# cosmir17/Scala-akka-tensorflow-sharetrade-helper

Hardware: AMD Instinct MI355X
Metric: env steps/sec (whole node) + episode return, 2x128 MLP Q-net at 1/2/4/8 MI355X (higher is better)
Workload: dtype bf16; 1 GPU; model=2x128 MLP Q-net (203->128->128->3), online DQN, Adam, global_batch=1835008, seq_len=201, parallelism=dp1, dp_gradient_sync=none, envs_per_gpu=1835008, hip_graph=True, graph_steps=16, kernel_chunk=64, step_kernel=ws, chunk_schedule=static

## Files before the change

### csrc/qstep_ws.hip

```cpp
#include "qstep.h"

#ifndef WS_STAMPS
#define WS_STAMPS 0
#endif
#ifndef WS_GSKIP
#define WS_GSKIP 0
#endif
#if WS_MARKS
#define WS_MARK(W, I) asm volatile(";@" #W " " #I);
#else
#define WS_MARK(W, I)
#endif
#ifndef WS_PD1
#define WS_PD1 8
#endif
#ifndef WS_NOPHIL
#define WS_NOPHIL 0
#endif
constexpr int WS_GXP = 2;
#ifndef WS_L2PRE
#define WS_L2PRE 4
#endif
#ifndef WS_WAIT_UNROLL
#define WS_WAIT_UNROLL -1
#endif
#ifndef WS_SLEEP
#define WS_SLEEP 1
#endif
#ifndef WS_ABORT_WORD
#define WS_ABORT_WORD 1
#endif
#ifndef WS_NOWB
#define WS_NOWB 0
#endif
#ifndef WS_NOPF
#define WS_NOPF 0
#endif
#ifndef WS_L1REP
#define WS_L1REP 1
#endif
#ifndef WS_L2REP
#define WS_L2REP 1
#endif
#ifndef WS_GST_MASK
#define WS_GST_MASK 0x7F
#endif
#ifndef WS_NS
#define WS_NS ws
#define WS_API(name) name
#endif

namespace st {
namespace WS_NS {

constexpr int NW = 8, NT = 64 * NW;
constexpr int ND = 4, NG = 4;
constexpr int C = 64;
constexpr int INP = 224, HP = 128;
constexpr int KX = 208;
constexpr int HWIN = 201;
constexpr int NSLOT = 4;
static_assert(NSLOT % ND == 0, "a data wave reuses its own slots (sequence q = ND k + d)");

constexpr int oW0 = 0;
constexpr int oW1 = oW0 + HP * KX * 2;
constexpr int oW2 = oW1 + HP * HP * 2;
constexpr int oB1 = oW2 + 5 * HP * 2;
constexpr int oB2 = oB1 + HP * 4;
constexpr int oSLOT = oB2 + 64;
constexpr int sX = 0, sH1 = sX + 16 * KX * 2, sH2 = sH1 + 16 * HP * 2, sDZ2 = sH2 + 16 * HP * 2,
              SLOT_BYTES = sDZ2 + 16 * HP * 2;
constexpr int oCTL = oSLOT + NSLOT * SLOT_BYTES;
constexpr int oST = oCTL + 64;
constexpr int LDS_BYTES = oST + ND * NSTAT * 4;
static_assert(LDS_BYTES <= 163840, "LDS budget");
static_assert(SLOT_BYTES % 16 == 0 && oSLOT % 16 == 0, "alignment");

ST_DEV int pi_pos4(int i, int q) { return 32 * (i >> 1) + 8 * q + 4 * (i & 1); }
ST_DEV int w1_off(int R, int s) { return R * HP + ((((s >> 3) ^ (2 * (R & 7)))) << 3) + (s & 7); }
ST_DEV int a_off(int r, int c) {
  return r * HP + ((((c >> 2) ^ ((4 * (r & 7)) | ((r >> 2) & 3)))) << 2) + (c & 3);
}

ST_DEV s8v zero_s8() { s8v z = {0, 0, 0, 0, 0, 0, 0, 0}; return z; }
ST_DEV s4v mask_bf(f4v v, s4v act) {
  return pk4(act[0] > 0 ? v[0] : 0.f, act[1] > 0 ? v[1] : 0.f, act[2] > 0 ? v[2] : 0.f, act[3] > 0 ? v[3] : 0.f);
}
ST_DEV s4v lo4(s8v v) { s4v r = {v[0], v[1], v[2], v[3]}; return r; }
ST_DEV s4v hi4(s8v v) { s4v r = {v[4], v[5], v[6], v[7]}; return r; }

#ifndef WS_PD2
#define WS_PD2 8
#endif
constexpr int PD2 = WS_PD2, NB2 = PD2 + 1;
template <int NPRE>
ST_DEV void layer2_pre(const bf16_t* W1p, int l16, int g4, s8v* A) {
#pragma unroll
  for (int j = 0; j < NPRE; ++j) A[j] = lds_ld8(W1p + w1_off(16 * (j & 7) + l16, 32 * (j >> 3) + 8 * g4));
}
template <int NPRE = 0>
ST_DEV void layer2(const bf16_t* W1p, int l16, int g4, const s8v* H, f4v* acc, const bf16_t* w2row, s8v* w2f,
                   const s8v* Apre = nullptr) {
  s8v A[NB2];
#pragma unroll
  for (int j = 0; j < NPRE; ++j) A[j] = Apre[j];
#pragma unroll
  for (int j = NPRE; j < PD2; ++j) A[j] = lds_ld8(W1p + w1_off(16 * (j & 7) + l16, 32 * (j >> 3) + 8 * g4));
  if (NPRE < PD2) __builtin_amdgcn_sched_group_barrier(0x100, PD2 - NPRE, 0);
#pragma unroll
  for (int j = 0; j < 32; ++j) {
    acc[j & 7] = mfma32(A[j % NB2], H[j >> 3], acc[j & 7]);
    __builtin_amdgcn_sched_group_barrier(0x008, 1, 0);
    if (j + PD2 < 32) {
      const int jn = j + PD2;
      A[jn % NB2] = lds_ld8(W1p + w1_off(16 * (jn & 7) + l16, 32 * (jn >> 3) + 8 * g4));
      __builtin_amdgcn_sched_group_barrier(0x100, 1, 0);
    } else if (j >= 32 - 4) {
      w2f[j - 28] = lds_ld8(w2row + 32 * (j - 28));
      __builtin_amdgcn_sched_group_barrier(0x100, 1, 0);
    }
  }
  __builtin_amdgcn_sched_barrier(0);
}

constexpr int SPIN_LIMIT = 1 << 24;
constexpr int CTL_ABORT = 12;
constexpr int CTL_NROUNDS = 13;
ST_DEV int cid_word(int r) { const int s = r & 3; return s == 0 ? 0 : (s == 1 ? 9 : (s == 2 ? 14 : 15)); }
constexpr int CID_SHIFT = 21, CID_MASK = (1 << CID_SHIFT) - 1;
ST_DEV void ws_fail(const QStepParams& p, int* ctl) {
  if ((threadIdx.x & 63) == 0) {
    __hip_atomic_store(ctl + CTL_ABORT, 1, __ATOMIC_RELAXED, __HIP_MEMORY_SCOPE_WORKGROUP);
    if (p.err != nullptr) atomicOr(p.err, 1u);
  }
}
template <typename Pred>
ST_DEV void ring_wait(const QStepParams& p, int* ctl, const int* w, Pred pred) {
#if WS_WAIT_UNROLL > 0
#pragma clang loop unroll_count(WS_WAIT_UNROLL)
#elif WS_WAIT_UNROLL == 0
#pragma clang loop unroll(disable)
#endif
  for (int spin = 0; !pred(lds_acq(w)); ++spin) {
    if (WS_ABORT_WORD && lds_acq(ctl + CTL_ABORT)) break;
    if (WS_SLEEP > 0) __builtin_amdgcn_s_sleep(WS_SLEEP);
    if (spin > SPIN_LIMIT) { ws_fail(p, ctl); break; }
  }
}

ST_DEV int* env_ptr(const QStepParams& p, int R, int e) {
  return reinterpret_cast<int*>(reinterpret_cast<char*>(p.env + (size_t)R * p.E) + (unsigned)e * 4u);
}
#undef ENV_I
#undef ENV_F
#define ENV_I(R, e) (*env_ptr(p, (R), (e)))
#define ENV_F(R, e) (*reinterpret_cast<float*>(env_ptr(p, (R), (e))))

ST_DEV bool wait_full_or_end(const QStepParams& p, int* ctl, int sa, int q) {
#pragma clang loop unroll(disable)
  for (int spin = 0;; ++spin) {
    if (lds_acq(ctl + 1 + sa) == q + 1) return false;
    const int n = lds_acq(ctl + CTL_NROUNDS);
    if (n != 0 && q / ND >= n - 1) return true;
    if (WS_ABORT_WORD && lds_acq(ctl + CTL_ABORT)) return true;
    __builtin_amdgcn_s_sleep(1);
    if (spin > SPIN_LIMIT) { ws_fail(p, ctl); return true; }
  }
}

template <int FEAT, bool DYN, bool KN, bool U16 = false>
__global__ void __launch_bounds__(NT, 1) qstep_ws_kernel(QStepParams p) {
  static_assert(!U16 || FEAT, "the tick bank serves the relative features (w / last - 1) only");
  extern __shared__ __attribute__((aligned(16))) char smem[];
  bf16_t* W0p = reinterpret_cast<bf16_t*>(smem + oW0);
  bf16_t* W1p = reinterpret_cast<bf16_t*>(smem + oW1);
  bf16_t* W2p = reinterpret_cast<bf16_t*>(smem + oW2);
  float* sB1 = reinterpret_cast<float*>(smem + oB1);
  float* sB2 = reinterpret_cast<float*>(smem + oB2);
  int* ctl = reinterpret_cast<int*>(smem + oCTL);
  float* sSt = reinterpret_cast<float*>(smem + oST);

  const int tid = threadIdx.x, lane = tid & 63, l16 = lane & 15, g4 = lane >> 4;
  const int wave = __builtin_amdgcn_readfirstlane(tid >> 6);
  const unsigned long long step = p.ctrl[0];
  const int nchunks = p.E / C;
  const int nmy = (nchunks - (int)blockIdx.x + (int)gridDim.x - 1) / (int)gridDim.x;
  const int xg = (int)blockIdx.x & 7, gx = (int)gridDim.x >> 3;
  auto static_chunk = [&](int k) {
    const int c = (int)blockIdx.x + k * (int)gridDim.x;
    return c < nchunks ? c : -1;
  };

#if defined(WS_PROLOGUE_REPS) && WS_PROLOGUE_REPS > 1
  for (int rep_ = 0; rep_ < WS_PROLOGUE_REPS; ++rep_) {
    __syncthreads();
#else
  {
#endif
   if (p.wimg != nullptr) {
    constexpr int NCH = (oSLOT - oW0) / 16;
    for (int j = wave; j * 64 < NCH; j += NT / 64) {
      const int c = j * 64 + lane;
      if (c < NCH)
        __builtin_amdgcn_global_load_lds((const __attribute__((address_space(1))) void*)(p.wimg + 16 * c),
                                         (__attribute__((address_space(3))) void*)(smem + oW0 + 1024 * j), 16, 0, 0);
    }
    __builtin_amdgcn_s_waitcnt(0xF70);
   } else {
    const bf16_t* w0 = p.wq + p.off_w0;
    for (int i = tid; i < HP * KX; i += NT) {
      const int r = i / KX, s = i % KX;
      W0p[i] = w0[r * INP + slot_col(s)];
    }
    const bf16_t* w1 = p.wq + p.off_w1;
    for (int i = tid; i < HP * HP; i += NT) {
      const int R = i >> 7, s = i & 127;
      W1p[w1_off(R, s)] = w1[R * HP + pi_unit(s)];
    }
    const bf16_t* w2 = p.wq + p.off_w2;
    for (int i = tid; i < 5 * HP; i += NT) {
      const int a = i >> 7, s = i & 127;
      W2p[i] = w2[a * HP + pi_unit(s)];
    }
    for (int i = tid; i < HP; i += NT) sB1[i] = p.wf[p.off_b1 + i];
    if (tid < 16) sB2[tid] = tid < 4 ? p.wf[p.off_b2 + tid] : 0.f;
   }
    if (tid < 16) ctl[tid] = 0;
    if (DYN && tid == 0) {
      int r = 0;
      while (r < 3 && static_chunk(r) >= 0) ++r;
      if (r < 3) ctl[CTL_NROUNDS] = r + 1;
    }
  }
  __syncthreads();

  if (wave < ND) {
    const int d = wave;
    float st_reward = 0.f, st_loss = 0.f, st_explore = 0.f, st_done = 0.f, st_fsum = 0.f, st_fsq = 0.f,
          st_qslot = 0.f;
    const float b2v[3] = {sB2[0], sB2[1], sB2[2]};

    int ck0 = DYN ? static_chunk(0) : (int)blockIdx.x, ck1 = DYN ? static_chunk(1) : 0, ck2 = DYN ? static_chunk(2) : 0;
    auto ring_chunk = [&](int r) {
      int v = 0;
      ring_wait(p, ctl, ctl + cid_word(r), [&](int w) { v = w; return (w >> CID_SHIFT) == (r & 0x3FF); });
      return (v & CID_MASK) - 1;
    };
    unsigned claim_v = 0u;
    bool claim_out = false, ended = DYN && ck2 < 0;
    unsigned* const head = DYN ? p.chunk_heads + 32 * xg : nullptr;
    auto env_of = [&](int k, int rel) {
      if (DYN) {
        const int c = rel == 0 ? ck0 : (rel == 1 ? ck1 : ck2);
        return max(c, 0) * C + 16 * d + l16;
      }
      return (min((int)blockIdx.x + k * (int)gridDim.x, nchunks - 1)) * C + 16 * d + l16;
    };
    int e_pos, e_sh, e_ep, n_pos, n_sh, n_ep;
    float e_b, e_val, e_rs, n_b, n_val, n_rs;
    float e_sc = 1.f, n_sc = 1.f;
#define WS_LOAD_ENV(K, REL, POS, B, SH, VAL, RS, EP, SC)                                          \
  {                                                                                              \
    const int e_ = env_of(K, REL);                                                               \
    POS = ENV_I(ER_POS, e_); B = ENV_F(ER_BUDGET, e_); SH = ENV_I(ER_SHARES, e_);                \
    VAL = ENV_F(ER_VALUE, e_); RS = ENV_F(ER_RET_SUM, e_); EP = ENV_I(ER_EPISODES, e_);          \
    if (U16) SC = p.tscale[e_];                                                                  \
  }
    float4 pa[6], pb[6];
    float pc[6];
    float4 pd = make_float4(0.f, 0.f, 0.f, 0.f);
    float pe = 0.f;
    float4 pl;
    uint4 ta[6];
    unsigned tb[6];
    uint2 td = make_uint2(0u, 0u);
    unsigned te = 0u;
    uint2 tl;
#define WS_LOAD_PRICES(K, REL, POS)                                                               \
  if (U16) {                                                                                     \
    const int e_ = env_of(K, REL);                                                               \
    const int pc_ = min(max((POS), 0), p.T - HWIN - 1);                                          \
    const unsigned* b_ = reinterpret_cast<const unsigned*>(p.ticks + (size_t)e_ * p.T16) + (pc_ >> 1); \
    __builtin_memcpy(&tl, b_ + 100, sizeof(tl));                                                 \
    _Pragma("unroll") for (int ks = 0; ks < 6; ++ks) {                                           \
      __builtin_memcpy(&ta[ks], b_ + 16 * ks + 4 * g4, sizeof(uint4));                           \
      tb[ks] = b_[16 * ks + 4 * g4 + 4];                                                         \
    }                                                                                            \
    if (g4 == 1 || g4 == 2) {                                                                    \
      __builtin_memcpy(&td, b_ + 94 + 2 * g4, sizeof(td));                                       \
      te = b_[96 + 2 * g4];                                                                      \
    }                                                                                            \
  } else {                                                                                       \
    const int e_ = env_of(K, REL);                                                               \
    const int pc_ = min(max((POS), 0), p.T - HWIN - 1);    \
    const float* b_ = p.prices4 + (size_t)e_ * p.T4 + (size_t)pc_;     \
    pl = ldu4(b_ + 200);                           \
    _Pragma("unroll") for (int ks = 0; ks < 6; ++ks) {                                           \
      const float* q_ = b_ + 32 * ks + 8 * g4;                                                   \
      pa[ks] = ldu4(q_);                                                                         \
      pb[ks] = ldu4(q_ + 4);                                                                     \
      pc[ks] = q_[8];                                                                            \
    }                                                                                            \
    if (g4 == 1 || g4 == 2) {                                                                    \
      const float* r_ = b_ + 188 + 4 * g4;                                                       \
      pd = ldu4(r_);                                                                             \
      pe = r_[4];                                                                                \
    }                                                                                            \
  }
    WS_LOAD_ENV(0, 0, e_pos, e_b, e_sh, e_val, e_rs, e_ep, e_sc)
    WS_LOAD_PRICES(0, 0, e_pos)
    WS_LOAD_ENV(1, 1, n_pos, n_b, n_sh, n_val, n_rs, n_ep, n_sc)

    unsigned long long* stamps = ((WS_STAMPS & 1) && p.stamps != nullptr && blockIdx.x == 0 && d == 0 && lane == 0)
                                     ? p.stamps : nullptr;
#define WS_STAMP(I) if ((WS_STAMPS & 1) && stamps) stamps[k * 16 + (I)] = __builtin_amdgcn_s_memtime(); WS_MARK(D, I)
#define WS_PIN(V) asm volatile("" ::"v"(V))
#define WS_SB() __builtin_amdgcn_sched_barrier(0)

    int w_e = -1, w_s = 0, w_pos = 0, w_ep = 0, w_act = 0;
    float w_b = 0.f, w_v = 0.f, w_rs = 0.f, w_fin = 0.f, w_rew = 0.f;
    bool w_done = false;
#define WS_WRITE_BACK()                                                                           \
  if (!WS_NOWB && g4 == 0 && w_e >= 0) {                                                         \
    ENV_F(ER_BUDGET, w_e) = w_b; ENV_I(ER_SHARES, w_e) = w_s; ENV_F(ER_VALUE, w_e) = w_v;        \
    ENV_I(ER_POS, w_e) = w_pos; ENV_F(ER_RET_SUM, w_e) = w_rs;                                   \
    ENV_I(ER_ACTION, w_e) = w_act; ENV_F(ER_REWARD, w_e) = w_rew;                                \
    if (w_done) { ENV_F(ER_LAST_FINAL, w_e) = w_fin; ENV_I(ER_EPISODES, w_e) = w_ep; }           \
  }
#define WS_WB_SET()                                                                               \
  {                                                                                              \
    const int np_ = pos + 1;                                                                     \
    w_e = e; w_act = act; w_rew = rew;                                                           \
    w_done = np_ >= p.T - HWIN;                                                                  \
    w_ep = w_done ? ep0 + 1 : ep0;                                                               \
    if (w_done) {                                                                                \
      w_fin = __fadd_rn(b2, __fmul_rn((float)s2, vnew));                                         \
      w_b = p.b0; w_s = p.s0; w_v = 0.f; w_pos = 0; w_rs = 0.f;                                  \
    } else {                                                                                     \
      w_b = b2; w_s = s2; w_v = vnew; w_pos = np_; w_rs = rs0 + rew;                             \
    }                                                                                            \
    WS_WRITE_BACK() w_e = -1;                                                                    \
  }

    for (int k = 0; DYN ? ck0 >= 0 : k < nmy; ++k) {
      WS_STAMP(0);
      const int chunk = DYN ? ck0 : (int)blockIdx.x + k * (int)gridDim.x;
      if (DYN && k >= 1) ck2 = __builtin_amdgcn_readfirstlane(ring_chunk(k + 2));
      const int e = chunk * C + 16 * d + l16;
      float lastw, vnew_w, last, vnew;
      unsigned shb = 0u;
      if (U16) {
        shb = (unsigned)(min(max(e_pos, 0), p.T - HWIN - 1) & 1) * 2u;
        const unsigned t01 = __builtin_amdgcn_alignbyte(tl.y, tl.x, shb);
        lastw = (float)(t01 & 0xFFFFu);
        vnew_w = (float)(t01 >> 16);
        last = __fmul_rn(lastw, e_sc);
        vnew = __fmul_rn(vnew_w, e_sc);
      } else {
        lastw = last = pl.x;
        vnew_w = vnew = pl.y;
      }
      float inv = 0.f, invn = 0.f;
      if (FEAT) {
        inv = __fdiv_rn(1.0f, lastw);
        invn = __fdiv_rn(1.0f, vnew_w);
      }
      auto fx = [&](float w) {
        return FEAT ? __fmaf_rn(w, inv, -1.0f) : w;
      };
      auto fxn = [&](float w) {
        return FEAT ? __fmaf_rn(w, invn, -1.0f) : w;
      };
      auto lo16f = [](unsigned v) { return (float)(v & 0xFFFFu); };
      auto hi16f = [](unsigned v) { return (float)(v >> 16); };
      s8v X[6], Xn[6];
#pragma unroll
      for (int ks = 0; ks < 6; ++ks) {
        if (U16) {
          const unsigned w0 = __builtin_amdgcn_alignbyte(ta[ks].y, ta[ks].x, shb),
                         w1 = __builtin_amdgcn_alignbyte(ta[ks].z, ta[ks].y, shb),
                         w2 = __builtin_amdgcn_alignbyte(ta[ks].w, ta[ks].z, shb),
                         w3 = __builtin_amdgcn_alignbyte(tb[ks], ta[ks].w, shb),
                         w4 = __builtin_amdgcn_alignbyte(0u, tb[ks], shb);
          const float f0 = lo16f(w0), f1 = hi16f(w0), f2 = lo16f(w1), f3 = hi16f(w1), f4 = lo16f(w2),
                      f5 = hi16f(w2), f6 = lo16f(w3), f7 = hi16f(w3), f8 = lo16f(w4);
          X[ks] = cat8(pk4(fx(f0), fx(f1), fx(f2), fx(f3)), pk4(fx(f4), fx(f5), fx(f6), fx(f7)));
          Xn[ks] = cat8(pk4(fxn(f1), fxn(f2), fxn(f3), fxn(f4)), pk4(fxn(f5), fxn(f6), fxn(f7), fxn(f8)));
        } else {
          X[ks] = cat8(pk4(fx(pa[ks].x), fx(pa[ks].y), fx(pa[ks].z), fx(pa[ks].w)),
                       pk4(fx(pb[ks].x), fx(pb[ks].y), fx(pb[ks].z), fx(pb[ks].w)));
          Xn[ks] = cat8(pk4(fxn(pa[ks].y), fxn(pa[ks].z), fxn(pa[ks].w), fxn(pb[ks].x)),
                        pk4(fxn(pb[ks].y), fxn(pb[ks].z), fxn(pb[ks].w), fxn(pc[ks])));
        }
      }
      s4v X6, Xn6;
      if (g4 == 0) {
        X6 = pk4(feat_budget(e_b, p.inv_b0, FEAT), feat_shares(e_sh, last, p.inv_b0, FEAT), 1.0f, fx(lastw));
        Xn6 = zero_s4();
      } else if (g4 < 3) {
        if (U16) {
          const unsigned v0 = __builtin_amdgcn_alignbyte(td.y, td.x, shb), v1 = __builtin_amdgcn_alignbyte(te, td.y, shb),
                         v2 = __builtin_amdgcn_alignbyte(0u, te, shb);
          const float f0 = lo16f(v0), f1 = hi16f(v0), f2 = lo16f(v1), f3 = hi16f(v1), f4 = lo16f(v2);
          X6 = pk4(fx(f0), fx(f1), fx(f2), fx(f3));
          Xn6 = pk4(fxn(f1), fxn(f2), fxn(f3), fxn(f4));
        } else {
          X6 = pk4(fx(pd.x), fx(pd.y), fx(pd.z), fx(pd.w));
          Xn6 = pk4(fxn(pd.y), fxn(pd.z), fxn(pd.w), fxn(pe));
        }
      } else {
        X6 = zero_s4();
        Xn6 = zero_s4();
      }
      const int pos = e_pos, sh0 = e_sh, ep0 = e_ep;
      const float bud0 = e_b, vprev = e_val, rs0 = e_rs;
      e_pos = n_pos; e_b = n_b; e_sh = n_sh; e_val = n_val; e_rs = n_rs; e_ep = n_ep; e_sc = n_sc;
      WS_PIN(X[5]); WS_PIN(Xn[5]); WS_PIN(X6);
      WS_SB();
      WS_STAMP(1);
      WS_WRITE_BACK()
      WS_LOAD_ENV(k + 2, 2, n_pos, n_b, n_sh, n_val, n_rs, n_ep, n_sc)
      if (DYN && d == 0 && !ended) {
        if (lane == 0) claim_v = atomicAdd(head, 1u);
        claim_out = true;
      }
      float u1 = u24((uint32_t)(p.env_offset + e)), u2 = u24((uint32_t)step);
      if (!WS_NOPHIL) policy_draw((uint32_t)(p.env_offset + e), step, p.key0, p.key1, u1, u2);
      f4v a1[8], a1n[8];
#pragma unroll
      for (int i = 0; i < 8; ++i) { a1[i] = zero4(); a1n[i] = zero4(); }
      {
        constexpr int PD1 = WS_PD1, NB1 = PD1 + 1;
        const bf16_t* w0b = W0p + l16 * KX + 8 * g4;
        for (int rep = 0; rep < WS_L1REP; ++rep) {
        s8v A[NB1];
#pragma unroll
        for (int j = 0; j < PD1; ++j) A[j] = lds_ld8(w0b + (j & 7) * 16 * KX + 32 * (j >> 3));
        __builtin_amdgcn_sched_group_barrier(0x100, PD1, 0);
#pragma unroll
        for (int j = 0; j < 48; ++j) {
          const int ks = j >> 3, i = j & 7;
          a1[i] = mfma32(A[j % NB1], X[ks], a1[i]);
          a1n[i] = mfma32(A[j % NB1], Xn[ks], a1n[i]);
          __builtin_amdgcn_sched_group_barrier(0x008, 2, 0);
          if (j + PD1 < 48) {
            const int jn = j + PD1;
            A[jn % NB1] = lds_ld8(w0b + (jn & 7) * 16 * KX + 32 * (jn >> 3));
            __builtin_amdgcn_sched_group_barrier(0x100, 1, 0);
          }
          __builtin_amdgcn_sched_group_barrier(0x002, 2, 0);
        }
        }
        WS_PIN(u1); WS_PIN(u2);
        WS_SB();
      }
      WS_STAMP(12);
      s4v w06[8];
#pragma unroll
      for (int i = 0; i < 8; ++i) {
        w06[i] = lds_ld4(W0p + (16 * i + l16) * KX + 192 + 4 * g4);
        a1[i] = mfma16(w06[i], X6, a1[i]);
      }
      s8v H1[4];
#pragma unroll
      for (int ks = 0; ks < 4; ++ks) H1[ks] = cat8(relu_bf(a1[2 * ks]), relu_bf(a1[2 * ks + 1]));
      f4v a2[8];
#pragma unroll
      for (int i = 0; i < 8; ++i) a2[i] = *reinterpret_cast<const f4v*>(sB1 + 16 * i + 4 * g4);
      WS_PIN(H1[3]); WS_PIN(a1n[7]);
      WS_SB();
      WS_STAMP(2);
      s8v A2pre[WS_L2PRE];
      layer2_pre<WS_L2PRE>(W1p, l16, g4, A2pre);
      const int q = ND * k + d;
      const int sl = q % NSLOT, round = q / NSLOT;
      ring_wait(p, ctl, ctl + 5 + sl, [&](int v) { return v >= NG * round; });
      WS_STAMP(3);
      char* sb = smem + oSLOT + sl * SLOT_BYTES;
      bf16_t* sx = reinterpret_cast<bf16_t*>(sb + sX);
      bf16_t* sh1 = reinterpret_cast<bf16_t*>(sb + sH1);
      bf16_t* sh2 = reinterpret_cast<bf16_t*>(sb + sH2);
      bf16_t* sz2 = reinterpret_cast<bf16_t*>(sb + sDZ2);
#pragma unroll
      for (int ks = 0; ks < 6; ++ks) *reinterpret_cast<s8v*>(sx + l16 * KX + 32 * ks + 8 * g4) = X[ks];
      if (g4 < 3) *reinterpret_cast<s4v*>(sx + l16 * KX + 192 + 4 * g4) = X6;
#pragma unroll
      for (int i = 0; i < 8; ++i)
        *reinterpret_cast<s4v*>(sh1 + a_off(l16, 16 * i + 4 * g4)) = (i & 1) ? hi4(H1[i >> 1]) : lo4(H1[i >> 1]);
      WS_SB();
      WS_STAMP(4);
      const bf16_t* w2row = W2p + min(l16, 4) * HP + 8 * g4;
      s8v w2f[4];
      layer2<WS_L2PRE>(W1p, l16, g4, H1, a2, w2row, w2f, A2pre);
      s8v H2[4];
#pragma unroll
      for (int ks = 0; ks < 4; ++ks) H2[ks] = cat8(relu_bf(a2[2 * ks]), relu_bf(a2[2 * ks + 1]));
#pragma unroll
      for (int i = 0; i < 8; ++i)
        *reinterpret_cast<s4v*>(sh2 + a_off(l16, 16 * i + 4 * g4)) = (i & 1) ? hi4(H2[i >> 1]) : lo4(H2[i >> 1]);
      WS_PIN(H2[3]);
      WS_SB();
      WS_STAMP(5);
      f4v qa = zero4();
#pragma unroll
      for (int ks = 0; ks < 4; ++ks) {
        const s8v a = w2f[ks];
        qa = mfma32(a, H2[ks], qa);
      }
      WS_PIN(qa);
      WS_SB();
      WS_STAMP(6);
      float b2 = 0.f, rew = 0.f, q0 = 0.f, q1 = 0.f, q2 = 0.f;
      int s2 = 0, act = 0;
      if (g4 == 0) {
        q0 = qa[0] + b2v[0];
        q1 = qa[1] + b2v[1];
        q2 = qa[2] + b2v[2];
        if (p.output_relu) { q0 = fmaxf(q0, 0.f); q1 = fmaxf(q1, 0.f); q2 = fmaxf(q2, 0.f); }
        const int greedy = argmax3(q0, q1, q2);
        const bool exploit = exploits(u1, p.eps, (KN && p.ramp_global) ? (float)step : (float)pos, p.inv_ramp);
        const int rnd = random_action(u2);
        act = exploit ? greedy : rnd;
        const Holding h2 = trade(act, trade_base(bud0, sh0, p.compat_env, p.b0, p.s0), vnew);
        b2 = h2.budget;
        s2 = h2.shares;
        rew = reward(bud0, sh0, vprev, b2, s2, vnew, p.reward_mode);
        Xn6 = pk4(feat_budget(b2, p.inv_b0, FEAT), feat_shares(s2, vnew, p.inv_b0, FEAT), 1.0f, fxn(vnew_w));
        st_explore += exploit ? 0.f : 1.f;
      }
      WS_WB_SET()
      WS_PIN(Xn6);
      WS_SB();
      WS_STAMP(7);
#pragma unroll
      for (int i = 0; i < 8; ++i) a1n[i] = mfma16(w06[i], Xn6, a1n[i]);
      s8v H1n[4];
#pragma unroll
      for (int ks = 0; ks < 4; ++ks) H1n[ks] = cat8(relu_bf(a1n[2 * ks]), relu_bf(a1n[2 * ks + 1]));
      WS_LOAD_PRICES(k + 1, 1, e_pos)
#pragma unroll
      for (int i = 0; i < 8; ++i) a2[i] = *reinterpret_cast<const f4v*>(sB1 + 16 * i + 4 * g4);
      WS_SB();
      for (int rep = 0; rep < WS_L2REP; ++rep) layer2(W1p, l16, g4, H1n, a2, w2row, w2f);
      s8v H2n[4];
#pragma unroll
      for (int ks = 0; ks < 4; ++ks) H2n[ks] = cat8(relu_bf(a2[2 * ks]), relu_bf(a2[2 * ks + 1]));
      f4v qn = zero4();
#pragma unroll
      for (int ks = 0; ks < 4; ++ks) {
        const s8v a = w2f[ks];
        qn = mfma32(a, H2n[ks], qn);
      }
      WS_PIN(qn);
      WS_SB();
      WS_STAMP(8);
      const bf16_t* zchunk = reinterpret_cast<const bf16_t*>(ctl + 10);
      s4v aw[8], h2m[8];
      auto dz_reads = [&]() {
// ... 7 lines not shown
      float dq = 0.f;
      int slot = 0;
      if (g4 == 0) {
        float4 tq = make_float4(0.f, 0.f, 0.f, 0.f);
        if (KN && p.qt != nullptr) tq = *reinterpret_cast<const float4*>(p.qt + ((size_t)e * 3 + act) * 4);
        float n0 = qn[0] + b2v[0], n1 = qn[1] + b2v[1], n2 = qn[2] + b2v[2];
        if (p.output_relu) { n0 = fmaxf(n0, 0.f); n1 = fmaxf(n1, 0.f); n2 = fmaxf(n2, 0.f); }
        float vnext;
        const int am = argmax3(n0, n1, n2, vnext);
        slot = p.target_compat ? am : act;
        if (KN && p.qt != nullptr) vnext = target_value(tq.x, tq.y, tq.z, am, p.target_compat || p.double_dqn);
        const float y = td_target(rew, KN ? p.reward_scale : 1.0f, p.gamma, vnext);
        const float qs = slot == 0 ? q0 : (slot == 1 ? q1 : q2);
        float diff;
        dq = td_dq(qs, y, p.loss_coef, p.td_clip, p.output_relu, diff);
        float fdone = 0.f, ndone = 0.f;
        if (pos + 1 >= p.T - HWIN) {
          fdone = __fadd_rn(b2, __fmul_rn((float)s2, vnew));
          ndone = 1.f;
        }
        st_reward += rew;
        st_loss += diff * diff;
        st_qslot += qs;
        st_done += ndone;
        st_fsum += fdone;
        st_fsq += fdone * fdone;
      }
      WS_SB();
      WS_STAMP(9);
      const s4v bq = g4 == 0 ? pk4(slot == 0 ? dq : 0.f, slot == 1 ? dq : 0.f, slot == 2 ? dq : 0.f, 0.f)
                             : zero_s4();
      s4v dz[8];
      f4v zt[8];
#pragma unroll
      for (int i = 0; i < 8; ++i) zt[i] = mfma16(aw[i], bq, zero4());
#pragma unroll
      for (int i = 0; i < 8; ++i) dz[i] = mask_pk(zt[i], h2m[i]);
      WS_PIN(dz[7]);
      WS_SB();
      WS_STAMP(10);
#pragma unroll
      for (int ks = 0; ks < 4; ++ks)
        *reinterpret_cast<s8v*>(sz2 + w1_off(l16, 32 * ks + 8 * g4)) = cat8(dz[2 * ks], dz[2 * ks + 1]);
      if (g4 == 0) *reinterpret_cast<s4v*>(sx + l16 * KX + 204) = bq;
      if (lane == 0) __hip_atomic_store(ctl + 1 + sl, q + 1, __ATOMIC_RELEASE, __HIP_MEMORY_SCOPE_WORKGROUP);
      if (DYN) {
        if (d == 0) {
          int c = -1;
          if (claim_out) {
            const unsigned cv = (unsigned)__builtin_amdgcn_readfirstlane((int)claim_v);
            const long long cc = 8ll * (3ll * gx + (long long)cv) + xg;
            c = cc < nchunks ? (int)cc : -1;
            claim_out = false;
          }
          const bool first_end = c < 0 && !ended;
          if (c < 0) ended = true;
          if (lane == 0) {
            if (first_end && ck2 >= 0)
              __hip_atomic_store(ctl + CTL_NROUNDS, k + 3 + 1, __ATOMIC_RELAXED, __HIP_MEMORY_SCOPE_WORKGROUP);
            __hip_atomic_store(ctl + cid_word(k + 3), (((k + 3) & 0x3FF) << CID_SHIFT) | (c + 1), __ATOMIC_RELEASE,
                               __HIP_MEMORY_SCOPE_WORKGROUP);
          }
        }
        ck0 = ck1;
        ck1 = ck2;
      }
      WS_SB();
      WS_STAMP(11);
    }
    WS_WRITE_BACK()
#undef WS_WRITE_BACK
#undef WS_WB_SET
#undef WS_LOAD_ENV
#undef WS_LOAD_PRICES
#undef WS_STAMP
    const float v[NSTAT - 1] = {st_reward, st_loss, st_explore, st_done, st_fsum, st_fsq, st_qslot};
#pragma unroll
    for (int s = 0; s < NSTAT - 1; ++s) {
      const float t = wave_sum(v[s]);
      if (lane == 0) sSt[d * NSTAT + s] = t;
    }
    if (lane == 0) sSt[d * NSTAT + NSTAT - 1] = 0.f;
    __syncthreads();
  } else {
    const int gw = wave - ND;
    f4v gW0[2][13], gW1[2][8], gW2[2];
    float gB1s[2] = {0.f, 0.f}, gB2s = 0.f;
    auto sum8 = [](const s8v& v) {
      float acc = 0.f;
#pragma unroll
      for (int j = 0; j < 8; ++j) acc += bf2f((bf16_t)v[j]);
      return acc;
    };
#pragma unroll
    for (int m = 0; m < 2; ++m) {
#pragma unroll
      for (int n = 0; n < 13; ++n) gW0[m][n] = zero4();
#pragma unroll
      for (int n = 0; n < 8; ++n) gW1[m][n] = zero4();
      gW2[m] = zero4();
    }
    s4v ones;
#pragma unroll
    for (int j = 0; j < 4; ++j) ones[j] = (l16 == 0) ? (short)0x3F80 : (short)0;
    const int r4 = 4 * g4 + (l16 >> 2), qq = l16 & 3;
    const bf16_t* zchunk = reinterpret_cast<const bf16_t*>(ctl + 10);
    const int nseq = ND * nmy;
    unsigned long long* gst = ((WS_STAMPS & 2) && p.stamps != nullptr && blockIdx.x == 0 && gw == 0 && lane == 0)
                                  ? p.stamps + (size_t)(nmy + 1) * 16 : nullptr;
    unsigned long long gts[7] = {0, 0, 0, 0, 0, 0, 0};
#define WS_GST(I) if ((WS_STAMPS & 2) && ((WS_GST_MASK >> (I)) & 1)) gts[I] = __builtin_amdgcn_s_memtime(); WS_MARK(G, I)
    int nseqv = DYN ? 0x7FFFFFF0 : nseq;
    for (int q = 0; q < nseqv; q += 2) {
      const int sa = q % NSLOT, sb = (q + 1) % NSLOT;
      WS_GST(0);
      if (DYN) {
        if (wait_full_or_end(p, ctl, sa, q)) {
          nseqv = q;
          continue;
        }
      } else {
        ring_wait(p, ctl, ctl + 1 + sa, [&](int v) { return v == q + 1; });
      }
      ring_wait(p, ctl, ctl + 1 + sb, [&](int v) { return v == q + 2; });
      WS_GST(1);
#if WS_GSKIP
      if (lane == 0) {
        __hip_atomic_fetch_add(ctl + 5 + sa, 1, __ATOMIC_RELEASE, __HIP_MEMORY_SCOPE_WORKGROUP);
        __hip_atomic_fetch_add(ctl + 5 + sb, 1, __ATOMIC_RELEASE, __HIP_MEMORY_SCOPE_WORKGROUP);
      }
      continue;
#endif
      const char* pa_ = smem + oSLOT + sa * SLOT_BYTES;
      const char* pb_ = smem + oSLOT + sb * SLOT_BYTES;
      const bf16_t *xa = reinterpret_cast<const bf16_t*>(pa_ + sX), *xb = reinterpret_cast<const bf16_t*>(pb_ + sX);
      const bf16_t *h1a = reinterpret_cast<const bf16_t*>(pa_ + sH1), *h1b = reinterpret_cast<const bf16_t*>(pb_ + sH1);
      const bf16_t *h2a = reinterpret_cast<const bf16_t*>(pa_ + sH2), *h2b = reinterpret_cast<const bf16_t*>(pb_ + sH2);
      const bf16_t *z2a = reinterpret_cast<const bf16_t*>(pa_ + sDZ2), *z2b = reinterpret_cast<const bf16_t*>(pb_ + sDZ2);
      auto tr8 = [&](const bf16_t* a, const bf16_t* b, int off) { return cat8(lds_tr4(a + off), lds_tr4(b + off)); };
      f4v c1a[2] = {zero4(), zero4()}, c1b[2] = {zero4(), zero4()};
#pragma unroll
      for (int ks = 0; ks < 4; ++ks) {
        const s8v aza = lds_ld8(z2a + w1_off(l16, 32 * ks + 8 * g4));
        const s8v azb = lds_ld8(z2b + w1_off(l16, 32 * ks + 8 * g4));
        const int R = 32 * ks + 4 * g4 + (l16 >> 2);
#pragma unroll
        for (int t = 0; t < 2; ++t) {
          const int col = pi_pos4(2 * gw + t, qq);
          const s8v wt = cat8(lds_tr4(W1p + w1_off(R, col)), lds_tr4(W1p + w1_off(R + 16, col)));
          c1a[t] = mfma32(aza, wt, c1a[t]);
          c1b[t] = mfma32(azb, wt, c1b[t]);
        }
      }
      s4v bowna[2], bownb[2];
#pragma unroll
      for (int t = 0; t < 2; ++t) {
        bowna[t] = lds_tr4(h1a + a_off(r4, 16 * (2 * gw + t) + 4 * qq));
        bownb[t] = lds_tr4(h1b + a_off(r4, 16 * (2 * gw + t) + 4 * qq));
      }
      constexpr int XD = WS_GXP;
      s8v bx[13];
#pragma unroll
      for (int n = 0; n < XD; ++n) bx[n] = tr8(xa, xb, r4 * KX + 16 * n + 4 * qq);
      WS_PIN(c1a[1]); WS_PIN(c1b[1]);
      WS_SB();
      WS_GST(2);
      s8v a0[2];
#pragma unroll
      for (int t = 0; t < 2; ++t) a0[t] = cat8(mask_pk(c1a[t], bowna[t]), mask_pk(c1b[t], bownb[t]));
      WS_PIN(a0[1]);
      WS_SB();
      WS_GST(3);
#pragma unroll
      for (int n = 0; n < 13; ++n) {
#pragma unroll
        for (int m = 0; m < 2; ++m) gW0[m][n] = mfma32(a0[m], bx[n], gW0[m][n]);
        __builtin_amdgcn_sched_group_barrier(0x008, 2, 0);
        if (n + XD < 13) {
          bx[n + XD] = tr8(xa, xb, r4 * KX + 16 * (n + XD) + 4 * qq);
          __builtin_amdgcn_sched_group_barrier(0x100, 2, 0);
        }
      }
      WS_PIN(gW0[1][12]);
      WS_SB();
      WS_GST(4);
      s8v a1[2];
#pragma unroll
      for (int m = 0; m < 2; ++m) a1[m] = tr8(z2a, z2b, w1_off(r4, pi_pos4(2 * gw + m, qq)));
#pragma unroll
      for (int m = 0; m < 2; ++m) gB1s[m] += sum8(a1[m]);
#pragma unroll
      for (int half = 0; half < 2; ++half) {
        s8v bh[4];
#pragma unroll
        for (int k = 0; k < 4; ++k) bh[k] = tr8(h1a, h1b, a_off(r4, 16 * (4 * half + k) + 4 * qq));
#pragma unroll
        for (int m = 0; m < 2; ++m)
#pragma unroll
          for (int k = 0; k < 4; ++k) gW1[m][4 * half + k] = mfma32(a1[m], bh[k], gW1[m][4 * half + k]);
      }
      {
        const s8v aq = qq == 0 ? tr8(xa, xb, r4 * KX + 204) : cat8(lds_tr4(zchunk), lds_tr4(zchunk));
        s8v bh2[2];
#pragma unroll
        for (int k = 0; k < 2; ++k) bh2[k] = tr8(h2a, h2b, a_off(r4, 16 * (2 * gw + k) + 4 * qq));
        if (lane == 0) {
          __hip_atomic_fetch_add(ctl + 5 + sa, 1, __ATOMIC_RELEASE, __HIP_MEMORY_SCOPE_WORKGROUP);
          __hip_atomic_fetch_add(ctl + 5 + sb, 1, __ATOMIC_RELEASE, __HIP_MEMORY_SCOPE_WORKGROUP);
        }
        WS_GST(5);
#pragma unroll
        for (int n = 0; n < 2; ++n) gW2[n] = mfma32(aq, bh2[n], gW2[n]);
        gB2s += sum8(aq);
      }
      WS_PIN(gW1[1][7]); WS_PIN(gB2s);
      WS_SB();
      WS_GST(6);
      if ((WS_STAMPS & 2) && gst) {
#pragma unroll
        for (int i = 0; i < 7; ++i) gst[8 * q + i] = gts[i];
      }
    }
    __syncthreads();
    auto put = [&](int idx, float v) {
      if (p.slab_bf16) {
        bf16_t* sbf = reinterpret_cast<bf16_t*>(p.slab);
        sbf[((size_t)(idx >> 5) * p.slab_rows + blockIdx.x) * 32 + (idx & 31)] = f2bf(v);
      } else {
        p.slab[(size_t)blockIdx.x * p.P + idx] = v;
      }
    };
#pragma unroll
    for (int m = 0; m < 2; ++m)
#pragma unroll
      for (int j = 0; j < 4; ++j) {
        const int u = 32 * gw + 16 * m + 4 * g4 + j;
#pragma unroll
        for (int n = 0; n < 13; ++n) put(p.off_w0 + u * INP + slot_col(16 * n + l16), gW0[m][n][j]);
#pragma unroll
        for (int n = 0; n < 8; ++n) put(p.off_w1 + u * HP + 16 * n + l16, gW1[m][n][j]);
      }
#pragma unroll
    for (int m = 0; m < 2; ++m) {
      float v = gB1s[m];
      v += __shfl_xor(v, 16, 64);
      v += __shfl_xor(v, 32, 64);
      if (g4 == 0) put(p.off_b1 + 32 * gw + 16 * m + l16, v);
    }
    {
      float v = gB2s;
      v += __shfl_xor(v, 16, 64);
      v += __shfl_xor(v, 32, 64);
      if (gw == 0 && g4 == 0 && l16 < 4) put(p.off_b2 + l16, v);
    }
#pragma unroll
    for (int n = 0; n < 2; ++n)
#pragma unroll
      for (int j = 0; j < 4; ++j) put(p.off_w2 + (4 * g4 + j) * HP + 16 * (2 * gw + n) + l16, gW2[n][j]);
  }
#undef WS_SB
#undef WS_PIN
#undef WS_GST
  if (tid < NSTAT) {
    float t = 0.f;
#pragma unroll
    for (int w = 0; w < ND; ++w) t += sSt[w * NSTAT + tid];
    p.stats[(size_t)blockIdx.x * NSTAT + tid] = t;
  }
  if (blockIdx.x == 0 && tid == 0) p.ctrl[1] = step + 1;
}

template <int FEAT, bool DYN, bool KN, bool U16 = false>
static hipError_t launch_f(const QStepParams& p, int grid, hipStream_t stream) {
  static bool attr = false;
  if (!attr) {
    hipError_t e = hipFuncSetAttribute((const void*)qstep_ws_kernel<FEAT, DYN, KN, U16>,
                                       hipFuncAttributeMaxDynamicSharedMemorySize, LDS_BYTES);
    if (e != hipSuccess) return e;
    attr = true;
  }
  hipLaunchKernelGGL((qstep_ws_kernel<FEAT, DYN, KN, U16>), dim3(grid), dim3(NT), LDS_BYTES, stream, p);
  return hipGetLastError();
}

__global__ void __launch_bounds__(256) ws_img_map_kernel(int* map, int off_w0, int off_w1, int off_w2, int off_b1,
                                                         int off_b2) {
  const int i = blockIdx.x * blockDim.x + threadIdx.x;
  if (i < HP * KX) map[off_w0 + (i / KX) * INP + slot_col(i % KX)] = oW0 / 2 + i;
  if (i < HP * HP) map[off_w1 + (i >> 7) * HP + pi_unit(i & 127)] = oW1 / 2 + w1_off(i >> 7, i & 127);
  if (i < 5 * HP) map[off_w2 + (i >> 7) * HP + pi_unit(i & 127)] = oW2 / 2 + i;
  if (i < HP) map[off_b1 + i] = -(oB1 / 4 + i) - 2;
  if (i < 4) map[off_b2 + i] = -(oB2 / 4 + i) - 2;
}

}
}

extern "C" int WS_API(st_qstep_ws_img_bytes)() { return st::WS_NS::oSLOT - st::WS_NS::oW0; }

extern "C" hipError_t WS_API(st_qstep_ws_img_map)(int* map, int off_w0, int off_w1, int off_w2, int off_b1, int off_b2,
                                                  hipStream_t stream) {
  using namespace st::WS_NS;
  static_assert(oW0 == 0 && (oSLOT - oW0) % 16 == 0, "image run");
  hipLaunchKernelGGL(ws_img_map_kernel, dim3((HP * KX + 255) / 256), dim3(256), 0, stream, map, off_w0, off_w1, off_w2,
                     off_b1, off_b2);
  return hipGetLastError();
}

extern "C" int WS_API(st_qstep_ws_lds_bytes)(int inp, int h1p, int h2p) {
  if (inp == st::WS_NS::INP && h1p == st::WS_NS::HP && h2p == st::WS_NS::HP) return st::WS_NS::LDS_BYTES;
  return -1;
}

extern "C" hipError_t WS_API(st_qstep_ws_launch)(const st::QStepParams* p, int inp, int h1p, int h2p, int grid,
                                                 hipStream_t stream) {
  using namespace st::WS_NS;
  if (inp != INP || h1p != HP || h2p != HP || p->H != HWIN) return hipErrorInvalidValue;
  if (p->E % C != 0 || grid < 1 || grid > p->E / C) return hipErrorInvalidValue;
  if (p->chunk_heads != nullptr && (grid % 8 != 0 || p->E / C >= (1 << CID_SHIFT) - 1)) return hipErrorInvalidValue;
  if (p->T < HWIN + 2 || p->T4 < p->T + 4) return hipErrorInvalidValue;
  if ((p->off_w0 | p->off_w1 | p->off_w2) & 7) return hipErrorInvalidValue;
  if (p->slab_bf16 && (p->slab_rows != grid || p->P % 32 != 0)) return hipErrorInvalidValue;
  const bool kn = p->qt != nullptr || p->reward_scale != 1.0f || p->ramp_global || p->double_dqn;
  if (p->ticks != nullptr) {
    if (!p->feat_mode || p->tscale == nullptr || p->T16 < p->T + 8 || p->T16 % 8) return hipErrorInvalidValue;
    if (kn) {
      if (p->chunk_heads != nullptr || (p->double_dqn && p->qt == nullptr)) return hipErrorInvalidValue;
      return launch_f<1, false, true, true>(*p, grid, stream);
    }
    if (p->chunk_heads != nullptr) return launch_f<1, true, false, true>(*p, grid, stream);
    return launch_f<1, false, false, true>(*p, grid, stream);
  }
  if (kn) {
    if (p->chunk_heads != nullptr || (p->double_dqn && p->qt == nullptr)) return hipErrorInvalidValue;
    return p->feat_mode ? launch_f<1, false, true>(*p, grid, stream) : launch_f<0, false, true>(*p, grid, stream);
  }
  if (p->chunk_heads != nullptr)
    return p->feat_mode ? launch_f<1, true, false>(*p, grid, stream) : launch_f<0, true, false>(*p, grid, stream);
  return p->feat_mode ? launch_f<1, false, false>(*p, grid, stream) : launch_f<0, false, false>(*p, grid, stream);
}
```

### sharetrade/ops/native.py

```python
from __future__ import annotations

import ctypes as C
import os
from typing import Optional

import torch

_HERE = os.path.dirname(os.path.abspath(__file__))
LIB_DIR = os.path.join(os.path.dirname(_HERE), "_native")
HIP_LIB_PATH = os.path.join(LIB_DIR, "libsharetrade_hip.so")

_lib: Optional[C.CDLL] = None


class NativeUnavailable(RuntimeError):
    pass


class QStepParams(C.Structure):
    _fields_ = [
        ("prices", C.c_void_p), ("prices4", C.c_void_p), ("env", C.c_void_p),
        ("wq", C.c_void_p), ("wf", C.c_void_p), ("slab", C.c_void_p), ("stats", C.c_void_p), ("ctrl", C.c_void_p),
        ("T", C.c_int), ("E", C.c_int), ("H", C.c_int), ("P", C.c_int), ("T4", C.c_int),
        ("off_w0", C.c_int), ("off_w1", C.c_int), ("off_b1", C.c_int), ("off_w2", C.c_int), ("off_b2", C.c_int),
        ("eps", C.c_float), ("inv_ramp", C.c_float), ("gamma", C.c_float), ("loss_coef", C.c_float),
        ("b0", C.c_float), ("inv_b0", C.c_float),
        ("s0", C.c_int), ("compat_env", C.c_int), ("target_compat", C.c_int), ("output_relu", C.c_int),
        ("feat_mode", C.c_int),
        ("key0", C.c_uint32), ("key1", C.c_uint32),
        ("env_offset", C.c_int),
        ("stamps", C.c_void_p),
        ("slab_bf16", C.c_int), ("slab_rows", C.c_int),
        ("chunk_heads", C.c_void_p),
        ("reward_mode", C.c_int), ("td_clip", C.c_float),
        ("err", C.c_void_p),
        ("reward_scale", C.c_float), ("ramp_global", C.c_int), ("qt", C.c_void_p), ("double_dqn", C.c_int),
        ("wimg", C.c_void_p),
        ("ticks", C.c_void_p), ("tscale", C.c_void_p), ("T16", C.c_int),
    ]


QTARGET_VARIANTS = {0: (4, 4), 1: (2, 8), 2: (1, 8), 3: (1, 16)}


class QTargetParams(C.Structure):
    _fields_ = [
        ("prices4", C.c_void_p), ("env", C.c_void_p), ("wt", C.c_void_p), ("qt", C.c_void_p),
        ("T", C.c_int), ("E", C.c_int), ("T4", C.c_int),
        ("off_w0", C.c_int), ("off_w1", C.c_int), ("off_b1", C.c_int), ("off_w2", C.c_int), ("off_b2", C.c_int),
        ("b0", C.c_float), ("inv_b0", C.c_float),
        ("s0", C.c_int), ("compat_env", C.c_int), ("output_relu", C.c_int), ("feat_mode", C.c_int),
        ("wimg", C.c_void_p),
        ("ticks", C.c_void_p), ("tscale", C.c_void_p), ("T16", C.c_int),
    ]


class OptimParams(C.Structure):
    _fields_ = [
        ("params", C.c_void_p), ("params_bf", C.c_void_p), ("mask", C.c_void_p), ("s1", C.c_void_p),
        ("s2", C.c_void_p), ("slab", C.c_void_p), ("grad", C.c_void_p), ("ctrl", C.c_void_p),
        ("stats", C.c_void_p), ("stat_acc", C.c_void_p),
        ("G", C.c_int), ("P", C.c_int), ("kind", C.c_int), ("mode", C.c_int), ("nstat", C.c_int),
        ("lr", C.c_float), ("beta1", C.c_float), ("beta2", C.c_float), ("eps", C.c_float), ("scale", C.c_float),
        ("tdelay", C.c_int), ("slab_bf16", C.c_int),
        ("chunk_heads", C.c_void_p),
        ("ema", C.c_void_p), ("ema_decay", C.c_float),
        ("img_map", C.c_void_p), ("img", C.c_void_p),
    ]


REWARD_MODES = {"absolute": 0, "relative": 1, "growth": 2}

ENV_ROWS = ("pos", "budget", "shares", "value", "ret_sum", "episodes", "last_final", "actions_out", "rewards_out")


AB_LIB_PATH = os.path.join(LIB_DIR, "libsharetrade_ab.so")
WRONG_RESULT_VARIANTS = frozenset({"gskip", "gskipst", "l1x2", "l2x2", "nopf", "nowb", "nophil"})
_ab_lib: Optional[C.CDLL] = None


def ab_builds_enabled() -> bool:
    return os.environ.get("SHARETRADE_AB_BUILDS", "") not in ("", "0")


def ab_lib() -> C.CDLL:
    global _ab_lib
    if not ab_builds_enabled():
        raise RuntimeError("timing / debug kernel builds are opt-in: set SHARETRADE_AB_BUILDS=1 and run "
                           "`python build.py --ab` (csrc/ab/*.hip -> libsharetrade_ab.so)")
    if _ab_lib is None:
        if not os.path.exists(AB_LIB_PATH):
            raise NativeUnavailable(f"{AB_LIB_PATH} not built: run `SHARETRADE_AB_BUILDS=1 python build.py`")
        lib()
        _ab_lib = C.CDLL(AB_LIB_PATH)
    return _ab_lib


def variant_launch(suffix: str, prefix: str = "st_qstep_ws_launch_"):
    if not ab_builds_enabled():
        bad = " (computes WRONG results by design)" if suffix in WRONG_RESULT_VARIANTS else ""
        raise RuntimeError(f"engine.step_variant={suffix!r}{bad} needs SHARETRADE_AB_BUILDS=1")
    fn = getattr(ab_lib(), prefix + suffix)
    fn.argtypes = [C.POINTER(QStepParams), C.c_int, C.c_int, C.c_int, C.c_int, C.c_void_p]
    fn.restype = C.c_int
    return fn


def available() -> bool:
    return os.path.exists(HIP_LIB_PATH)


def lib() -> C.CDLL:
    global _lib
    if _lib is not None:
        return _lib
    if not os.path.exists(HIP_LIB_PATH):
        raise NativeUnavailable(
            f"{HIP_LIB_PATH} not built: run `python build.py` (hipcc --offload-arch=gfx950)")
    L = C.CDLL(HIP_LIB_PATH)
    L.st_qstep_launch.argtypes = [C.POINTER(QStepParams), C.c_int, C.c_int, C.c_int, C.c_int, C.c_void_p]
    L.st_qstep_launch.restype = C.c_int
    L.st_qstep_lds_bytes.argtypes = [C.c_int, C.c_int, C.c_int]
    L.st_qstep_lds_bytes.restype = C.c_int
    L.st_qstep_wide_launch.argtypes = [C.POINTER(QStepParams), C.c_int, C.c_int, C.c_int, C.c_int, C.c_void_p]
    L.st_qstep_wide_launch.restype = C.c_int
    L.st_qstep_wide_lds_bytes.argtypes = [C.c_int, C.c_int, C.c_int]
    L.st_qstep_wide_lds_bytes.restype = C.c_int
    L.st_qstep_wide_launch_w8.argtypes = [C.POINTER(QStepParams), C.c_int, C.c_int, C.c_int, C.c_int, C.c_void_p]
    L.st_qstep_wide_launch_w8.restype = C.c_int
    L.st_qstep_ws_launch.argtypes = [C.POINTER(QStepParams), C.c_int, C.c_int, C.c_int, C.c_int, C.c_void_p]
    L.st_qstep_ws_launch.restype = C.c_int
    L.st_qstep_ws_lds_bytes.argtypes = [C.c_int, C.c_int, C.c_int]
    L.st_qstep_ws_lds_bytes.restype = C.c_int
    L.st_qtarget_launch.argtypes = [C.POINTER(QTargetParams), C.c_int, C.c_void_p]
    L.st_qtarget_launch.restype = C.c_int
    L.st_qtarget_launch_v.argtypes = [C.POINTER(QTargetParams), C.c_int, C.c_int, C.c_void_p]
    L.st_qtarget_launch_v.restype = C.c_int
    L.st_qtarget_img_bytes.argtypes = []
    L.st_qtarget_img_bytes.restype = C.c_int
    L.st_qtarget_img_map.argtypes = [C.c_void_p] + [C.c_int] * 4 + [C.c_void_p]
    L.st_qtarget_img_map.restype = C.c_int
    L.st_f32b_target_sync.argtypes = [C.c_void_p, C.c_void_p, C.c_longlong, C.c_void_p, C.c_longlong, C.c_void_p]
    L.st_f32b_target_sync.restype = C.c_int
    L.st_reduce_optim.argtypes = [C.POINTER(OptimParams), C.c_void_p]
    L.st_reduce_optim.restype = C.c_int
    L.st_advance.argtypes = [C.c_void_p, C.c_void_p]
    L.st_advance.restype = C.c_int
    L.st_commit_step.argtypes = [C.c_void_p, C.c_void_p]
    L.st_commit_step.restype = C.c_int
    L.st_to_bf16.argtypes = [C.c_void_p, C.c_void_p, C.c_int, C.c_void_p]
    L.st_to_bf16.restype = C.c_int
    L.st_img_pack.argtypes = [C.c_void_p, C.c_void_p, C.c_void_p, C.c_int, C.c_void_p]
    L.st_img_pack.restype = C.c_int
    L.st_qstep_ws_img_bytes.argtypes = []
    L.st_qstep_ws_img_bytes.restype = C.c_int
    L.st_qstep_ws_img_map.argtypes = [C.c_void_p] + [C.c_int] * 5 + [C.c_void_p]
    L.st_qstep_ws_img_map.restype = C.c_int
    L.st_random_walk.argtypes = [C.c_void_p, C.c_int, C.c_int, C.c_float, C.c_float, C.c_float, C.c_uint32,
                                 C.c_uint32, C.c_void_p]
    L.st_random_walk.restype = C.c_int
# ... 151 lines not shown
```

Baseline: 3.083 billion env_steps/s.

## Stage gradient slab writeout through LDS for coalesced 16-byte bf16 stores

The gradient waves used to write per-block gradients straight to the bf16 slab as scattered 2-byte stores. They now pack values in padded LDS and then copy them out with coalesced uint4 stores in the slab's 32-column interleaved layout. The data waves add matching barriers, and the slot index is rewritten equivalently. This aims to cut the cost of the end-of-kernel writeback, at the price of extra syncthreads, an LDS zero-fill and reuse of the slot region. It also adds A/B builds (nowo, dskip) that skip the writeout or the data work for timing.

```diff
diff --git a/csrc/ab/qstep_ws_dskip.hip b/csrc/ab/qstep_ws_dskip.hip
--- /dev/null
+++ b/csrc/ab/qstep_ws_dskip.hip
@@ -0,0 +1,4 @@
+#define WS_DSKIP 1
+#define WS_NS ws_dskip
+#define WS_API(name) name##_dskip
+#include "../qstep_ws.hip"
diff --git a/csrc/ab/qstep_ws_nowo.hip b/csrc/ab/qstep_ws_nowo.hip
--- /dev/null
+++ b/csrc/ab/qstep_ws_nowo.hip
@@ -0,0 +1,4 @@
+#define WS_NOWO 1
+#define WS_NS ws_nowo
+#define WS_API(name) name##_nowo
+#include "../qstep_ws.hip"
diff --git a/csrc/qstep_ws.hip b/csrc/qstep_ws.hip
--- a/csrc/qstep_ws.hip
+++ b/csrc/qstep_ws.hip
@@ -32,6 +32,12 @@
 #endif
 #ifndef WS_NOWB
 #define WS_NOWB 0
+#endif
+#ifndef WS_NOWO
+#define WS_NOWO 0
+#endif
+#ifndef WS_DSKIP
+#define WS_DSKIP 0
 #endif
 #ifndef WS_NOPF
 #define WS_NOPF 0
@@ -76,6 +82,12 @@
 static_assert(LDS_BYTES <= 163840, "LDS budget");
 static_assert(SLOT_BYTES % 16 == 0 && oSLOT % 16 == 0, "alignment");
 
+constexpr int WO_PAD = 32, WO_NPAD = 2 * (HP / 4);
+ST_DEV int wo_off(int idx, int off_w0, int off_w1) {
+  const int g = idx < off_w1 ? min(max(idx - off_w0, 0) / (4 * INP), HP / 4) : HP / 4 + min((idx - off_w1) / (4 * HP), HP / 4);
+  return 2 * idx + WO_PAD * g;
+}
+
 ST_DEV int pi_pos4(int i, int q) { return 32 * (i >> 1) + 8 * q + 4 * (i & 1); }
 ST_DEV int w1_off(int R, int s) { return R * HP + ((((s >> 3) ^ (2 * (R & 7)))) << 3) + (s & 7); }
 ST_DEV int a_off(int r, int c) {
@@ -233,6 +245,13 @@
     }
   }
   __syncthreads();
+
+  const bool wo_lds = !WS_NOWO && p.slab_bf16;
+  constexpr int NTG = 64 * NG;
+  auto wo_zero_fill = [&]() {
+    const int nb = 2 * p.P + WO_PAD * WO_NPAD;
+    for (int o = 16 * (tid - 64 * ND); o < nb; o += 16 * NTG) *reinterpret_cast<uint4*>(smem + o) = make_uint4(0u, 0u, 0u, 0u);
+  };
 
   if (wave < ND) {
     const int d = wave;
@@ -342,7 +361,7 @@
     WS_WRITE_BACK() w_e = -1;                                                                    \
   }
 
-    for (int k = 0; DYN ? ck0 >= 0 : k < nmy; ++k) {
+    for (int k = 0; !WS_DSKIP && (DYN ? ck0 >= 0 : k < nmy); ++k) {
       WS_STAMP(0);
       const int chunk = DYN ? ck0 : (int)blockIdx.x + k * (int)gridDim.x;
       if (DYN && k >= 1) ck2 = __builtin_amdgcn_readfirstlane(ring_chunk(k + 2));
@@ -473,7 +492,7 @@
       s8v A2pre[WS_L2PRE];
       layer2_pre<WS_L2PRE>(W1p, l16, g4, A2pre);
       const int q = ND * k + d;
-      const int sl = q % NSLOT, round = q / NSLOT;
+      const int sl = (ND * (k % (NSLOT / ND)) + d) % NSLOT, round = q / NSLOT;
       ring_wait(p, ctl, ctl + 5 + sl, [&](int v) { return v >= NG * round; });
       WS_STAMP(3);
       char* sb = smem + oSLOT + sl * SLOT_BYTES;
@@ -647,6 +666,10 @@
     }
     if (lane == 0) sSt[d * NSTAT + NSTAT - 1] = 0.f;
     __syncthreads();
+    if (wo_lds) {
+      __syncthreads();
+      __syncthreads();
+    }
   } else {
     const int gw = wave - ND;
     f4v gW0[2][13], gW1[2][8], gW2[2];
@@ -675,7 +698,7 @@
                                   ? p.stamps + (size_t)(nmy + 1) * 16 : nullptr;
     unsigned long long gts[7] = {0, 0, 0, 0, 0, 0, 0};
 #define WS_GST(I) if ((WS_STAMPS & 2) && ((WS_GST_MASK >> (I)) & 1)) gts[I] = __builtin_amdgcn_s_memtime(); WS_MARK(G, I)
-    int nseqv = DYN ? 0x7FFFFFF0 : nseq;
+    int nseqv = WS_DSKIP ? 0 : (DYN ? 0x7FFFFFF0 : nseq);
     for (int q = 0; q < nseqv; q += 2) {
       const int sa = q % NSLOT, sb = (q + 1) % NSLOT;
       WS_GST(0);
@@ -787,41 +810,86 @@
       }
     }
     __syncthreads();
-    auto put = [&](int idx, float v) {
-      if (p.slab_bf16) {
-        bf16_t* sbf = reinterpret_cast<bf16_t*>(p.slab);
-        sbf[((size_t)(idx >> 5) * p.slab_rows + blockIdx.x) * 32 + (idx & 31)] = f2bf(v);
-      } else {
-        p.slab[(size_t)blockIdx.x * p.P + idx] = v;
-      }
-    };
-#pragma unroll
-    for (int m = 0; m < 2; ++m)
-#pragma unroll
-      for (int j = 0; j < 4; ++j) {
-        const int u = 32 * gw + 16 * m + 4 * g4 + j;
-#pragma unroll
-        for (int n = 0; n < 13; ++n) put(p.off_w0 + u * INP + slot_col(16 * n + l16), gW0[m][n][j]);
-#pragma unroll
-        for (int n = 0; n < 8; ++n) put(p.off_w1 + u * HP + 16 * n + l16, gW1[m][n][j]);
-      }
+    if (wo_lds) {
+      wo_zero_fill();
+      __syncthreads();
+    }
+    const int u0 = 32 * gw + 4 * g4, pad0 = WO_PAD * (8 * gw + g4);
+    const int bw0 = 2 * (p.off_w0 + u0 * INP) + pad0;
+    const int bw1 = 2 * (p.off_w1 + u0 * HP) + pad0 + WO_PAD * (HP / 4);
+    const int brest = WO_PAD * WO_NPAD;
+    const int c12 = slot_col(192 + l16);
+    float b1v[2], b2v_;
 #pragma unroll
     for (int m = 0; m < 2; ++m) {
       float v = gB1s[m];
       v += __shfl_xor(v, 16, 64);
       v += __shfl_xor(v, 32, 64);
-      if (g4 == 0) put(p.off_b1 + 32 * gw + 16 * m + l16, v);
+      b1v[m] = v;
     }
     {
       float v = gB2s;
       v += __shfl_xor(v, 16, 64);
       v += __shfl_xor(v, 32, 64);
-      if (gw == 0 && g4 == 0 && l16 < 4) put(p.off_b2 + l16, v);
-    }
-#pragma unroll
-    for (int n = 0; n < 2; ++n)
-#pragma unroll
-      for (int j = 0; j < 4; ++j) put(p.off_w2 + (4 * g4 + j) * HP + 16 * (2 * gw + n) + l16, gW2[n][j]);
+      b2v_ = v;
+    }
+    auto write_out = [&](auto put2, auto put1) {
+#pragma unroll
+      for (int m = 0; m < 2; ++m)
+#pragma unroll
+        for (int j = 0; j < 4; j += 2) {
+          const int u = 32 * gw + 16 * m + 4 * g4 + j;
+          const int r0 = 2 * (16 * m + j) * INP + WO_PAD * 4 * m, r1 = 2 * (16 * m + j) * HP + WO_PAD * 4 * m;
+#pragma unroll
+          for (int n = 0; n < 12; ++n)
+            put2(bw0 + 2 * l16 + r0 + 32 * n, p.off_w0 + u * INP + 16 * n + l16, gW0[m][n][j],
+                 bw0 + 2 * l16 + r0 + 2 * INP + 32 * n, p.off_w0 + (u + 1) * INP + 16 * n + l16, gW0[m][n][j + 1]);
+          put2(bw0 + 2 * c12 + r0, p.off_w0 + u * INP + c12, gW0[m][12][j],
+               bw0 + 2 * c12 + r0 + 2 * INP, p.off_w0 + (u + 1) * INP + c12, gW0[m][12][j + 1]);
+#pragma unroll
+          for (int n = 0; n < 8; ++n)
+            put2(bw1 + 2 * l16 + r1 + 32 * n, p.off_w1 + u * HP + 16 * n + l16, gW1[m][n][j],
+                 bw1 + 2 * l16 + r1 + 2 * HP + 32 * n, p.off_w1 + (u + 1) * HP + 16 * n + l16, gW1[m][n][j + 1]);
+        }
+      if (g4 == 0) {
+        const int idx = p.off_b1 + 32 * gw + l16;
+        put2(2 * idx + brest, idx, b1v[0], 2 * (idx + 16) + brest, idx + 16, b1v[1]);
+      }
+      if (gw == 0 && g4 == 0 && l16 < 4) put1(2 * (p.off_b2 + l16) + brest, p.off_b2 + l16, b2v_);
+#pragma unroll
+      for (int n = 0; n < 2; ++n)
+#pragma unroll
+        for (int j = 0; j < 4; j += 2) {
+          const int idx = p.off_w2 + (4 * g4 + j) * HP + 16 * (2 * gw + n) + l16;
+          put2(2 * idx + brest, idx, gW2[n][j], 2 * (idx + HP) + brest, idx + HP, gW2[n][j + 1]);
+        }
+    };
+    if (WS_NOWO) {
+      write_out([&](int, int, float a, int, int, float b) { WS_PIN(a); WS_PIN(b); }, [&](int, int, float a) { WS_PIN(a); });
+    } else if (wo_lds) {
+      write_out(
+          [&](int oa, int, float a, int ob, int, float b) {
+            const uint32_t w = pack_bf2(a, b);
+            *reinterpret_cast<bf16_t*>(smem + oa) = (bf16_t)(w & 0xFFFFu);
+            *reinterpret_cast<bf16_t*>(smem + ob) = (bf16_t)(w >> 16);
+          },
+          [&](int oa, int, float a) { *reinterpret_cast<bf16_t*>(smem + oa) = f2bf(a); });
+    } else {
+      float* const row = p.slab + (size_t)blockIdx.x * p.P;
+      write_out([&](int, int ia, float a, int, int ib, float b) { row[ia] = a; row[ib] = b; },
+                [&](int, int ia, float a) { row[ia] = a; });
+    }
+    if (wo_lds) {
+      __syncthreads();
+      char* const gb = reinterpret_cast<char*>(p.slab) + (size_t)blockIdx.x * 64;
+      const unsigned blockb = (unsigned)p.slab_rows * 64u;
+      const int np = p.P >> 3;
+#pragma unroll 4
+      for (int i = tid - 64 * ND; i < np; i += NTG) {
+        const uint4 v = *reinterpret_cast<const uint4*>(smem + wo_off(8 * i, p.off_w0, p.off_w1));
+        *reinterpret_cast<uint4*>(gb + ((unsigned)(i >> 2) * blockb + (unsigned)(i & 3) * 16u)) = v;
+      }
+    }
   }
 #undef WS_SB
 #undef WS_PIN
@@ -886,6 +954,12 @@
   if (p->T < HWIN + 2 || p->T4 < p->T + 4) return hipErrorInvalidValue;
   if ((p->off_w0 | p->off_w1 | p->off_w2) & 7) return hipErrorInvalidValue;
   if (p->slab_bf16 && (p->slab_rows != grid || p->P % 32 != 0)) return hipErrorInvalidValue;
+  if (p->slab_bf16) {
+    const int rest = p->off_w1 + HP * HP;
+    if (2 * (long long)p->P + WO_PAD * WO_NPAD > oCTL || p->off_w0 < 0 || p->off_w0 + HP * INP > p->off_w1 ||
+        p->off_b1 < rest || p->off_w2 < rest || p->off_b2 < rest || 2ll * p->P * p->slab_rows >= (1ll << 32))
+      return hipErrorInvalidValue;
+  }
   const bool kn = p->qt != nullptr || p->reward_scale != 1.0f || p->ramp_global || p->double_dqn;
   if (p->ticks != nullptr) {
     if (!p->feat_mode || p->tscale == nullptr || p->T16 < p->T + 8 || p->T16 % 8) return hipErrorInvalidValue;
diff --git a/sharetrade/ops/native.py b/sharetrade/ops/native.py
--- a/sharetrade/ops/native.py
+++ b/sharetrade/ops/native.py
@@ -75,7 +75,7 @@
 
 
 AB_LIB_PATH = os.path.join(LIB_DIR, "libsharetrade_ab.so")
-WRONG_RESULT_VARIANTS = frozenset({"gskip", "gskipst", "l1x2", "l2x2", "nopf", "nowb", "nophil"})
+WRONG_RESULT_VARIANTS = frozenset({"gskip", "gskipst", "l1x2", "l2x2", "nopf", "nowb", "nophil", "nowo", "dskip"})
 _ab_lib: Optional[C.CDLL] = None
 
 
```

Result: no change. 3.099 billion env_steps/s (median of 6 runs) (+0.5%).
